# Pyrokine/LineSegmentDetector-SLAM

Measured on NVIDIA B200. Metric: lsd_source_mpixel_per_s, higher is better.
Workload: dtype f64

## Files before the change

include/lsdb200.h:

```cpp
#ifndef LSDB200_H
#define LSDB200_H
#include <stdint.h>

#ifdef __cplusplus
extern "C" {
#endif

#define LSDB_OK 0
#define LSDB_ERR_CUDA 1
#define LSDB_ERR_ARG 2
#define LSDB_ERR_CAPACITY 3
#define LSDB_ERR_TIMEOUT 4
#define LSDB_ERR_NO_DEVICE 5

#define LSDB_MAX_ANGLE 524288.0

typedef struct lsdb_ctx lsdb_ctx;
typedef struct lsdb_batch lsdb_batch;
typedef struct lsdb_fa_map lsdb_fa_map;

typedef struct {
    double sca;
    double sig;
    double angThre;
    double denThre;
    int pseBin;
    int _pad;
} lsdb_lsd_params;

typedef struct {
    double k, b, dx, dy, x1, y1, x2, y2, len;
    int orient;
    int _pad;
} lsdb_line;

typedef struct {
    double x1, y1, x2, y2, wid, cX, cY, deg, dx, dy, p, prec, logNFA;
} lsdb_rect;

enum { LSDB_STAGE_STENCIL = 0, LSDB_STAGE_ORDER = 1, LSDB_STAGE_GROW = 2, LSDB_NSTAGES = 3 };

typedef struct {
    long long cells, live_seeds, grows, grown_px, small, regrows, rrr_passes, nfa_calls, nfa_px,
        rejects, accepts, spec_evals, respec_evals, chunks;
    long long cyc_grow, cyc_rect, cyc_nfa, cyc_wait, cyc_retire, cyc_spec, cyc_respec;
    long long cyc_map, ns_map, spare_;
    long long rs_none, rs_conflict, rs_commit, rs_lost_commit, rs_pad[4];
} lsdb_stats;

int lsdb_create(lsdb_ctx** out, int device, void* stream);
int lsdb_set_team_warps(lsdb_ctx* ctx, int warps);
void lsdb_destroy(lsdb_ctx* ctx);
const char* lsdb_last_error(const lsdb_ctx* ctx);
const char* lsdb_version(void);

int lsdb_batch_create(lsdb_ctx* ctx, int n_maps, const int* cols, const int* rows,
                      const lsdb_lsd_params* params, int max_lines_per_map, lsdb_batch** out);
void lsdb_batch_destroy(lsdb_batch* b);
int lsdb_batch_upload(lsdb_batch* b, const uint8_t* const* maps);
int lsdb_batch_run(lsdb_batch* b);
int lsdb_batch_sync(lsdb_batch* b);
int lsdb_batch_download(lsdb_batch* b, int* counts, lsdb_line* lines, lsdb_rect* rects);
int lsdb_batch_line_image(lsdb_batch* b, int i, uint8_t* line_im);
int lsdb_batch_line_images(lsdb_batch* b, uint8_t* const* line_ims);
int lsdb_batch_planes(lsdb_batch* b, int i, double* mag, double* deg, uint8_t* used, int32_t* labels,
                      int32_t* seeds, int max_seeds, int* n_seeds, double* max_grad);
int lsdb_batch_stage_ms(lsdb_batch* b, float* ms );
int lsdb_batch_stats(lsdb_batch* b, lsdb_stats* total);
int lsdb_batch_map_stats(lsdb_batch* b, int i, lsdb_stats* out);
int lsdb_batch_launches(const lsdb_batch* b);
// ... 100 lines not shown
```

linesegmentdetector-slam_b200/__init__.py:

```python
import ctypes as C
import os
import numpy as np

HERE = os.path.dirname(os.path.abspath(__file__))
SO_PATH = os.path.join(HERE, "liblsdb200.so")
LSD_DEFAULTS = dict(sca=0.3, sig=0.6, angThre=22.5, denThre=0.7, pseBin=1024)
ERR_NAMES = {1: "CUDA", 2: "ARG", 3: "CAPACITY", 4: "TIMEOUT", 5: "NO_DEVICE"}
STAGES = ("stencil", "order", "grow")
STAT_FIELDS = ["cells", "live_seeds", "grows", "grown_px", "small", "regrows", "rrr_passes", "nfa_calls", "nfa_px",
               "rejects", "accepts", "spec_evals", "respec_evals", "chunks", "cyc_grow", "cyc_rect", "cyc_nfa", "cyc_wait",
               "cyc_retire", "cyc_spec", "cyc_respec", "cyc_map", "ns_map", "spare_", "rs_none", "rs_conflict", "rs_commit", "rs_lost_commit", "rs_pad0", "rs_pad1", "rs_pad2", "rs_pad3"]

LINE_DTYPE = np.dtype([("k", "f8"), ("b", "f8"), ("dx", "f8"), ("dy", "f8"), ("x1", "f8"), ("y1", "f8"), ("x2", "f8"),
                       ("y2", "f8"), ("len", "f8"), ("orient", "i4"), ("_pad", "i4")])
RECT_FIELDS = ["x1", "y1", "x2", "y2", "wid", "cX", "cY", "deg", "dx", "dy", "p", "prec", "logNFA"]
EST_DTYPE = np.dtype([("n_hyp", "i4"), ("n_kept", "i4"), ("best_x", "f8"), ("best_y", "f8"), ("best_ang", "f8"), ("best_score", "f8"),
                      ("mean_x", "f8"), ("mean_y", "f8"), ("mean_ang", "f8"), ("mean_score", "f8")])
SCAN_INFO_DTYPE = np.dtype([("n_lines", "i4"), ("n_pts", "i4"), ("im_cols", "i4"), ("im_rows", "i4"), ("lidar_x", "f8"), ("lidar_y", "f8")])
RDP_DEFAULTS = dict(least_point=3, thre_line=0.08, least_dist_m=0.5)
HYP_DTYPE = np.dtype([("frame", "i4"), ("i_scan", "i4"), ("i_map", "i4"), ("i_pair", "i4"), ("x", "f8"), ("y", "f8"),
                      ("ang", "f8"), ("score", "f8")])
LEGACY_EST_DTYPE = np.dtype([("n_cols", "i4"), ("best_col", "i4"), ("best_score", "f8"), ("estimate_pose", "f8", (3,)),
                             ("estimate_pose_realworld", "f8", (3,))])


class LsdbError(RuntimeError):
    pass


class _Params(C.Structure):
    _fields_ = [("sca", C.c_double), ("sig", C.c_double), ("angThre", C.c_double), ("denThre", C.c_double),
                ("pseBin", C.c_int), ("_pad", C.c_int)]


# ... 510 lines not shown
```

linesegmentdetector-slam_b200/csrc/api.cu:

```cuda
#include "../../include/lsdb200.h"
#include "lsdb_common.cuh"

#include <limits.h>
#include <stdio.h>
#include <stdlib.h>
#include <string.h>
#include <algorithm>
#include <math.h>
#include <string>
#include <vector>

struct lsdb_ctx {
    int device;
    cudaStream_t stream;
    bool ownStream;
    std::string err;
    double* lgammaTab;
    int lgammaN;
    int maxGrowCtas;
    int teamWarps;
    lsdb_batch* cached;
    cudaEvent_t faEv[2];
    float faMs;
    void* faDev; size_t faDevCap;
    void* faHost; size_t faHostCap;
    void* faAux; void* faAuxHost; size_t faAuxCap;
    void* faIn; size_t faInCap;
    void* faInHost; size_t faInHostCap;
    void* faKeep; size_t faKeepCap;
    void* fsOut; void* fsOutHost; size_t fsOutCap, fsOutHostCap;
    void* fsLinesDev; void* fsPtsDev;
    void* fsIm; size_t fsImCap;
    void* fsTmp; size_t fsTmpCap;
    float fsMs;
};

struct lsdb_batch {
    lsdb_ctx* ctx;
    int n;
    lsdb_lsd_params params;
    int maxSeg, listCap, arenaCap, nTiles, nCtas, nWarps, runAhead, bmCapWords, steal, stencilMode;
    size_t totalN, totalSrc, totalBan;
    std::vector<LsdbImg> imgs;
    LsdbLsdConst kc;
    uint8_t* src; double* mag; double* deg; double* cosm; double* sinm; unsigned int* state; unsigned short* bins; unsigned int* cells;
    int* labels; LsdbRect* rects; LsdbImgDyn* dyn; LsdbImg* imgsD; int* tileImg; unsigned int* lists;
    int* imgCounter; LsdbLsdConst* kcD; double* gaussDbg; unsigned char* recBuf; unsigned int* banBits;
    uint8_t* lineImD;
    double* mcCache;
    unsigned int* nzBits; int2* bandOf; int2* bandsOfImg; unsigned int* orderTabs; int nBands;
    LsdbImgDyn* dynH; LsdbRect* rectsH;
    cudaEvent_t ev[4];
    bool ran, downloaded, mcReady;
    int launches;
};

static int fail(lsdb_ctx* c, int code, const char* fmt, const char* a = "", long long v = 0) {
    char buf[512];
    snprintf(buf, sizeof buf, fmt, a, v);
    if (c) c->err = buf;
    return code;
}
#define CK(ctx, call)                                                                         \
    do {                                                                                      \
// ... 180 lines not shown
        int sms = 148;
        cudaDeviceGetAttribute(&sms, cudaDevAttrMultiProcessorCount, ctx->device);
        int bmMax = lsdb_grow_max_bitmap_words(ctx->device);
        int bmLimit = 48 * 1024 / 4;
        if (getenv("LSDB_SMEM_BAN_KB")) bmLimit = atoi(getenv("LSDB_SMEM_BAN_KB")) * 1024 / 4;
        if (bmMax > bmLimit) bmMax = bmLimit;
        b->bmCapWords = maxBanWords <= bmMax ? maxBanWords : 0;
        if (getenv("LSDB_NO_SMEM_BAN")) b->bmCapWords = 0;
        int nw = 1184 / n;
        if (nw > LSDB_GROW_WARPS) nw = LSDB_GROW_WARPS;
        const int sizeCap = maxN < 30000 ? 4 : 8;
        if (nw > sizeCap) nw = sizeCap;
        if (nw < 1) nw = 1;
        if (ctx->teamWarps > 0) nw = ctx->teamWarps;
        if (getenv("LSDB_GROW_WARPS")) { int v = atoi(getenv("LSDB_GROW_WARPS")); if (v >= 1 && v <= LSDB_GROW_WARPS) nw = v; }
        b->nWarps = nw;
        if (nw == 1 && !getenv("LSDB_SMEM_BAN_KB")) b->bmCapWords = 0;
        b->runAhead = 0;
        if (getenv("LSDB_RUNAHEAD")) b->runAhead = atoi(getenv("LSDB_RUNAHEAD"));
        b->stencilMode = lsdb_stencil_mode();
        b->steal = 0;
        if (getenv("LSDB_STEAL")) b->steal = atoi(getenv("LSDB_STEAL")) & 0xff;
        if (getenv("LSDB_SUPER_SHIFT")) b->steal |= ((atoi(getenv("LSDB_SUPER_SHIFT")) & 3) + 1) << 8;
        const int maxCtas = lsdb_grow_max_ctas(ctx->device, nw, b->bmCapWords);
        b->nCtas = n < maxCtas ? n : maxCtas;
        if (getenv("LSDB_GROW_CTAS")) { int v = atoi(getenv("LSDB_GROW_CTAS")); if (v >= 1 && v < b->nCtas) b->nCtas = v; }
        (void)sms;
    }

    cudaError_t e = cudaSuccess;
#define AL(ptr, bytes) if (e == cudaSuccess) e = cudaMalloc((void**)&(ptr), (bytes))
    AL(b->src, b->totalSrc + 64); AL(b->mag, b->totalN * 8); AL(b->deg, b->totalN * 8); AL(b->cosm, b->totalN * 16 + 16);    AL(b->state, b->totalN * 4);
    AL(b->bins, b->totalN * 2); AL(b->cells, b->totalN * 4); AL(b->labels, b->totalN * 4);
    AL(b->rects, (size_t)n * b->maxSeg * sizeof(LsdbRect)); AL(b->dyn, (size_t)n * sizeof(LsdbImgDyn));
    AL(b->imgsD, (size_t)n * sizeof(LsdbImg)); AL(b->tileImg, (size_t)b->nTiles * sizeof(int));
    b->arenaCap = 8 * b->listCap < (1 << 14) ? (1 << 14) : (8 * b->listCap > (1 << 16) ? (1 << 16) : 8 * b->listCap);
    AL(b->lists, (size_t)b->nCtas * lsdb_grow_words_per_cta(b->listCap, b->arenaCap, b->nWarps) * 4);
    AL(b->recBuf, (size_t)b->nCtas * lsdb_grow_rec_bytes_per_cta());
    AL(b->imgCounter, 64); AL(b->kcD, sizeof(LsdbLsdConst)); AL(b->banBits, (b->totalBan + 4) * 4); AL(b->nzBits, (b->totalBan + 4) * 4);
    std::vector<int2> bandOfH, bandsOfImgH(n);
    {
        int sms = 148;
        cudaDeviceGetAttribute(&sms, cudaDevAttrMultiProcessorCount, ctx->device);
        int K = (12 * sms + n - 1) / n;
        for (int i = 0; i < n; i++) {
            int k = K;
// ... 33 lines not shown
    for (int i = 0; i < b->n; i++) {
        const LsdbImg& im = b->imgs[i];
        CK(ctx, cudaMemcpy2DAsync(b->src + im.srcOff, im.srcPitch, maps[i], im.cols, im.cols, im.rows, cudaMemcpyHostToDevice, ctx->stream));
    }
    return LSDB_OK;
}

extern "C" int lsdb_batch_run(lsdb_batch* b) {
    if (!b) return LSDB_ERR_ARG;
    lsdb_ctx* ctx = b->ctx;
    cudaStream_t s = ctx->stream;
    CK(ctx, cudaSetDevice(ctx->device));
    CK(ctx, cudaMemsetAsync(b->dyn, 0, (size_t)b->n * sizeof(LsdbImgDyn), s));
    CK(ctx, cudaMemsetAsync(b->labels, 0, b->totalN * 4, s));
    CK(ctx, cudaMemsetAsync(b->imgCounter, 0, 64, s));
    CK(ctx, cudaEventRecord(b->ev[0], s));
    const int nStencil = lsdb_launch_stencil(s, b->nTiles, b->imgsD, b->tileImg, b->dyn, b->kcD, b->src, b->mag, b->deg, b->cosm, b->sinm, b->state, b->banBits, b->nzBits, b->gaussDbg, 0,
                        b->cells, b->totalN * 4, b->imgCounter + 8, b->stencilMode);
    CK(ctx, cudaEventRecord(b->ev[1], s));
    lsdb_launch_order(s, b->n, b->nBands, b->imgsD, b->dyn, b->kcD, b->mag, b->nzBits, b->bandOf, b->bandsOfImg, b->orderTabs, b->bins, b->cells);
    CK(ctx, cudaEventRecord(b->ev[2], s));
    lsdb_launch_grow(s, b->n, b->nCtas, b->nWarps, b->imgsD, b->dyn, b->kcD, b->mag, b->deg, b->cosm, b->sinm, b->state, b->cells, b->labels, b->rects,
                     b->maxSeg, b->lists, b->listCap, b->arenaCap, b->runAhead, b->recBuf, ctx->lgammaTab, ctx->lgammaN, b->imgCounter, b->banBits,
                     b->bmCapWords, b->steal);
    CK(ctx, cudaEventRecord(b->ev[3], s));
    CK(ctx, cudaGetLastError());
    b->ran = true; b->downloaded = false; b->launches = 4 + nStencil;
    return LSDB_OK;
}

extern "C" int lsdb_batch_launches(const lsdb_batch* b) { return b ? b->launches : 0; }

extern "C" int lsdb_batch_run_stencil_rows(lsdb_batch* b, int tileRow0, int tileRow1) {
    if (!b) return LSDB_ERR_ARG;
    lsdb_ctx* ctx = b->ctx;
    if (b->n != 1) return fail(ctx, LSDB_ERR_ARG, "lsdb_batch_run_stencil_rows: single-map batches only%s");
    const LsdbImg& im = b->imgs[0];
    if (tileRow0 < 0 || tileRow1 > im.tilesY || tileRow0 > tileRow1) return fail(ctx, LSDB_ERR_ARG, "lsdb_batch_run_stencil_rows: bad tile-row range%s");
    cudaStream_t s = ctx->stream;
    CK(ctx, cudaSetDevice(ctx->device));
    CK(ctx, cudaMemsetAsync(b->dyn, 0, sizeof(LsdbImgDyn), s));
    CK(ctx, cudaMemsetAsync(b->labels, 0, b->totalN * 4, s));
    CK(ctx, cudaMemsetAsync(b->imgCounter, 0, 64, s));
    CK(ctx, cudaEventRecord(b->ev[0], s));
    const int nStencil = lsdb_launch_stencil(s, (tileRow1 - tileRow0) * im.tilesX, b->imgsD, b->tileImg, b->dyn, b->kcD, b->src, b->mag, b->deg, b->cosm, b->sinm, b->state,
                        b->banBits, b->nzBits, b->gaussDbg, tileRow0 * im.tilesX, b->cells, b->totalN * 4, b->imgCounter + 8, b->stencilMode);
    CK(ctx, cudaEventRecord(b->ev[1], s));
// ... 17 lines not shown
    const LsdbImg& im = b->imgs[0];
    ptrs[0] = b->mag + im.nOff; rowBytes[0] = 8ll * im.W;
    ptrs[1] = b->deg + im.nOff; rowBytes[1] = 8ll * im.W;
    ptrs[2] = b->cosm + 2 * im.nOff; rowBytes[2] = 16ll * im.W;
    ptrs[3] = b->state + im.nOff; rowBytes[3] = 4ll * im.W;
    ptrs[4] = b->banBits + im.banOff; rowBytes[4] = 4ll * im.pw;
    ptrs[5] = b->nzBits + im.banOff; rowBytes[5] = 4ll * im.pw;
    *nPlanes = 6;
    if (tileRows) *tileRows = im.tilesY;
    if (rowsPerTile) *rowsPerTile = LSDB_TILE;
    return LSDB_OK;
}

extern "C" int lsdb_batch_run_regions(lsdb_batch* b) {
    if (!b) return LSDB_ERR_ARG;
    lsdb_ctx* ctx = b->ctx;
    cudaStream_t s = ctx->stream;
    CK(ctx, cudaSetDevice(ctx->device));
    CK(ctx, cudaEventRecord(b->ev[1], s));
    lsdb_launch_order(s, b->n, b->nBands, b->imgsD, b->dyn, b->kcD, b->mag, b->nzBits, b->bandOf, b->bandsOfImg, b->orderTabs, b->bins, b->cells);
    CK(ctx, cudaEventRecord(b->ev[2], s));
    lsdb_launch_grow(s, b->n, b->nCtas, b->nWarps, b->imgsD, b->dyn, b->kcD, b->mag, b->deg, b->cosm, b->sinm, b->state, b->cells, b->labels, b->rects,
                     b->maxSeg, b->lists, b->listCap, b->arenaCap, b->runAhead, b->recBuf, ctx->lgammaTab, ctx->lgammaN, b->imgCounter, b->banBits,
                     b->bmCapWords, b->steal);
    CK(ctx, cudaEventRecord(b->ev[3], s));
    CK(ctx, cudaGetLastError());
    b->ran = true; b->downloaded = false; b->launches += 4;
    return LSDB_OK;
}

static int fetch_dyn(lsdb_batch* b) {
    lsdb_ctx* ctx = b->ctx;
    CK(ctx, cudaSetDevice(ctx->device));
    CK(ctx, cudaMemcpyAsync(b->dynH, b->dyn, (size_t)b->n * sizeof(LsdbImgDyn), cudaMemcpyDeviceToHost, ctx->stream));
    CK(ctx, cudaStreamSynchronize(ctx->stream));
    for (int i = 0; i < b->n; i++) {
        if (b->dynH[i].err == LSDB_ERR_TIMEOUT) return fail(ctx, LSDB_ERR_TIMEOUT, "map %s%lld: ordered-commit watchdog fired", "", i);
        if (b->dynH[i].err) return fail(ctx, LSDB_ERR_CAPACITY, "map %s%lld: region list or segment capacity exceeded", "", i);
    }
    return LSDB_OK;
}

extern "C" int lsdb_batch_sync(lsdb_batch* b) {
    if (!b) return LSDB_ERR_ARG;
    if (!b->ran) return fail(b->ctx, LSDB_ERR_ARG, "lsdb_batch_sync before lsdb_batch_run%s");
    return fetch_dyn(b);
}
// ... 805 lines not shown
```

linesegmentdetector-slam_b200/csrc/grow.cu:

```cuda
#include "lsdb_common.cuh"
#include "../../include/lsdb200.h"
#include <stdlib.h>

#define NW_MAX LSDB_GROW_WARPS
#define ARENA_HDR 32
#define GRID 32
#define FULL 0xffffffffu

enum { OC_NONE = 0, OC_NOCHANGE = 1, OC_REJECT = 2, OC_ACCEPT = 3, OC_DEFER = 4 };
enum { ST_CELLS = 0, ST_LIVE, ST_GROWS, ST_GROWNPX, ST_SMALL, ST_REGROWS, ST_RRR, ST_NFACALLS, ST_NFAPX, ST_REJECTS,
       ST_ACCEPTS, ST_SPEC, ST_RESPEC, ST_CHUNKS, ST_N,
       TM_GROW = ST_N, TM_RECT, TM_NFA, TM_WAIT, TM_RETIRE, TM_SPEC, TM_RESPEC, TM_MAPCYC, TM_MAPNS, TM_SPARE, RS_NONE, RS_CONFLICT, RS_COMMIT, RS_LOST, RS_P0, RS_P1, RS_P2, RS_P3, TM_N };

#define RING 512
#define NSLOTS (RING / LSDB_SUPER)
#define LQ_CAP 256
#define SG_CAP 32
struct GrowShared {
    volatile int frontier;
    int nextChunk;
    int runAhead;
    int supShift;
    int retireLock;
    volatile int nSeg;
    volatile int abortFlag;
    int img;
    int nChunks;
    int nCells;
    volatile int chunkFlag[RING];
    volatile unsigned char chunkHeavy[RING];
    volatile int chunkSeen[RING];
    unsigned int slotHead[NSLOTS];
    volatile int slotPending[NSLOTS];
    volatile unsigned int lq[LQ_CAP][2];
    volatile unsigned int lqReady[LQ_CAP];
// ... 36 lines not shown
    const double* cosm;
    const double* sinm;
    unsigned int* list;
    unsigned int* scratch;
    unsigned int* arenas;
    unsigned int* q;
    int listCap, arenaCap;
    const LsdbLsdConst* kc;
    const double* lgammaTab;
    int lgammaN;
    GrowShared* sh;
    unsigned int* rej[2];
    int rejCap;
    unsigned int* pnd;
    int npnd;
    int steal;
    int specChunk;
    double* stage;
    volatile unsigned int* bm;
    bool bmInSmem;
    int pw;
    double logNT, regThre;
    int cellShift;
};

__device__ __forceinline__ void bbox_add(const WarpCtx& c, BBox& b, int x, int y) {
    b.x0 = min(b.x0, x); b.y0 = min(b.y0, y); b.x1 = max(b.x1, x); b.y1 = max(b.y1, y);
}

__device__ __noinline__ double d_sin(double x) { return lsdm_sin(x); }
__device__ __noinline__ double d_cos(double x) { return lsdm_cos(x); }
__device__ __noinline__ double d_atan2(double y, double x) { return lsdm_atan2(y, x); }
__device__ __noinline__ double d_log(double x) { return lsdm_log(x); }
__device__ __noinline__ double d_log10(double x) { return lsdm_log10(x); }
__device__ __noinline__ double d_exp(double x) { return lsdm_exp(x); }
__device__ __noinline__ double d_pow(double x, double y) { return lsdm_pow(x, y); }

__device__ __forceinline__ unsigned int pack_xy(int x, int y) { return ((unsigned int)y << 16) | (unsigned int)x; }
__device__ __forceinline__ int px_of(unsigned int v) { return (int)(v & 0xffffu); }
__device__ __forceinline__ int py_of(unsigned int v) { return (int)(v >> 16); }


__device__ void clear_bits(const WarpCtx& c, const unsigned int* lst, int num) {
    for (int k = c.lane; k < num; k += 32) {
        unsigned int v = lst[k];
        atomicAnd(&c.state[(size_t)py_of(v) * c.W + px_of(v)], ~c.mybit);
// ... 366 lines not shown
                        if (pass) {
                            lst[num] = pk;
                            rej[num] = 0;
                            num++;
                            mine |= sg_bit(n, m);
                            cosS += cd;
                            sinS += sd;
                            if (num >= T) running = false;
                            else {
                                n2 = cosS * cosS + sinS * sinS;
                                c2n2 = c2 * n2; m2 = 4e-13 * n2; nrmOK = n2 > 1e-18;
                            }
                        } else {
                            nr |= 1u << nb;
                        }
                    }
                }
            }
        }
    }
    return num;
}

__device__ __noinline__ Rect rect_from_region(const WarpCtx& c, const unsigned int* lst, int num, double regDeg, double aliPro,
                                 double degThre) {
    const int W = c.W;
    const double pi = c.kc->pi;
    TIC;
    double* stg = c.stage;
    double acc = 0.0;
    for (int base = 0; base < num; base += 32) {
        const int k = base + c.lane;
        const unsigned int v = k < num ? lst[k] : 0u;
        const double wv = k < num ? c.mag[(size_t)py_of(v) * W + px_of(v)] : 0.0;
        stg[c.lane * 4 + 0] = wv * px_of(v);
        stg[c.lane * 4 + 1] = wv * py_of(v);
        stg[c.lane * 4 + 2] = wv;
        __syncwarp();
        const int cnt = min(32, num - base);
        if (c.lane < 3)
            for (int j = 0; j < cnt; j++) acc += stg[j * 4 + c.lane];
        __syncwarp();
    }
    double cenX = __shfl_sync(FULL, acc, 0), cenY = __shfl_sync(FULL, acc, 1), weiSum = __shfl_sync(FULL, acc, 2);
    cenX = cenX / weiSum;
    cenY = cenY / weiSum;
// ... 554 lines not shown
    GrowShared& sh = *c.sh;
    unsigned int p = 0, ci = 0;
    int got = 0;
    if (c.lane == 0) {
        while (true) {
            const unsigned int h = *(volatile unsigned int*)&sh.lqHead;
            if (h == *(volatile unsigned int*)&sh.lqTail) break;
            const int e = h & (LQ_CAP - 1);
            if (sh.lqReady[e] != h + 1) break;
            p = sh.lq[e][0]; ci = sh.lq[e][1];
            if (atomicCAS(&sh.lqHead, h, h + 1) == h) { got = 1; break; }
        }
    }
    got = __shfl_sync(FULL, got, 0);
    if (!got) return false;
    p = __shfl_sync(FULL, p, 0); ci = __shfl_sync(FULL, ci, 0);
    eval_large(c, (int)p, (int)ci, R);
    __threadfence();
    if (c.lane == 0) atomicSub((int*)&sh.slotPending[slot_of_chunk(sh, (int)ci >> 5)], 1);
    __syncwarp();
    return true;
}

__device__ void speculate_super(WarpCtx& c, int chunk0, int nSub, const unsigned int* cl, int nCells, const ChunkRecs& R, int T) {
    GrowShared& sh = *c.sh;
    const int lane = c.lane;
    const unsigned int lt = (1u << lane) - 1u;
    long long tSpec = clock64();
    const int slot = slot_of_chunk(*c.sh, chunk0);
    unsigned int* q = c.q;
    int qn = 0;
    for (int s = 0; s < nSub; s++) {
        const int ci = (chunk0 + s) * LSDB_CHUNK + lane;
        const int p = ci < nCells ? (int)cl[ci] : -1;
        const bool live = p >= 0 && !seed_taken(lsdb_ld_state(&c.state[p]), chunk0 + s);
        const unsigned int bal = __ballot_sync(FULL, live);
        if (live) {
            const int k = qn + __popc(bal & lt);
            q[2 * k] = (unsigned int)p;
            q[2 * k + 1] = (unsigned int)((s << 5) | lane);
        }
        qn += __popc(bal);
        R.oc[(size_t)((chunk0 + s) & (RING - 1)) * 32 + lane] = OC_NONE;
    }
    if (lane < nSub) { sh.chunkHeavy[(chunk0 + lane) & (RING - 1)] = 0; sh.chunkSeen[(chunk0 + lane) & (RING - 1)] = -1; }
    __syncwarp();
    for (int base = 0; base < qn && !aborted(c); base += 32) {
        const int k = base + lane;
        bool act = k < qn;
        const unsigned int rel = act ? q[2 * k + 1] : 0u;
        const int myChunk = chunk0 + (int)(rel >> 5);
        const int myp = act ? (int)q[2 * k] : 0;
        if (act && seed_taken(lsdb_ld_state(&c.state[myp]), myChunk)) act = false;
        unsigned int lst[SG_CAP];
        unsigned int pnd[SG_PND];
        int num = 0, npnd = 0;
        bool large = act;
        const int L0 = sh.nSeg;
        __threadfence_block();
        if (T <= SG_CAP && c.kc->degThre <= c.kc->pi / 2.0) {
            num = small_grow(c, act, myp, T, lst, myChunk, pnd, npnd);
            large = act && num >= T;
        }
        __syncwarp();
        const bool small = act && !large && npnd >= 0;
        const int need = small ? num + npnd : 0;
        int incl = need;
#pragma unroll
        for (int o = 1; o < 32; o <<= 1) {
            const int t = __shfl_up_sync(FULL, incl, o);
            if (lane >= o) incl += t;
        }
        const int tot = __shfl_sync(FULL, incl, 31);
        const int off = tot > 0 ? slot_alloc(c, slot, tot) : -1;
        if (small && off >= 0) {
            const size_t ri = (size_t)(myChunk & (RING - 1)) * 32 + (rel & 31u);
            BBox sb; sb.x0 = sb.y0 = 0x7fffffff; sb.x1 = sb.y1 = -1;
            const int mine = off + (incl - need);
            unsigned int* dst = c.arenas + (size_t)slot * c.arenaCap + mine;
            for (int j = 0; j < num; j++) { dst[j] = lst[j]; bbox_add(c, sb, px_of(lst[j]), py_of(lst[j])); }
            for (int j = 0; j < npnd; j++) dst[num + j] = pnd[j];
            R.L0[ri] = L0; R.b0[ri] = pack_xy(sb.x0, sb.y0); R.b1[ri] = pack_xy(sb.x1, sb.y1); 
            R.off[ri] = 0; R.chk[ri] = num; R.chkOff[ri] = (unsigned int)mine;
            R.pnd[ri] = npnd; R.pndOff[ri] = (unsigned int)(mine + num);
// ... 221 lines not shown
            atomicAdd(&sh.stats[ST_CHUNKS], 1ull);
            __threadfence_block();
            sh.frontier = f + 1;
        }
        __syncwarp();
    }
    if (c.lane == 0) {
        atomicAdd(&sh.stats[TM_RETIRE], (unsigned long long)(clock64() - t0));
        __threadfence_block();
        atomicExch(&sh.retireLock, 0);
    }
    __syncwarp();
}

template <int MAXT>
__global__ void __launch_bounds__(MAXT, 1) lsdb_grow_kernel(int nImgs, const LsdbImg* __restrict__ imgs, LsdbImgDyn* __restrict__ dyn,
                                                                   const LsdbLsdConst* __restrict__ kc, const double* __restrict__ mag,
                                                                   const double* __restrict__ deg, const double* __restrict__ cosm,
                                                                   const double* __restrict__ sinm, unsigned int* __restrict__ state,
                                                                   const unsigned int* __restrict__ cells, int* __restrict__ labels,
                                                                   LsdbRect* __restrict__ rects, int maxSeg, unsigned int* __restrict__ lists,
                                                                   int listCap, int arenaCap, int runAhead, unsigned char* __restrict__ recBuf,
                                                                   const double* __restrict__ lgammaTab, int lgammaN, int* __restrict__ imgCounter,
                                                                   unsigned int* banBits, int bmCapWords, int steal) {
    __shared__ GrowShared sh;
    extern __shared__ unsigned int bmShared[];
    const int tid = threadIdx.x, lane = tid & 31, w = tid >> 5, nw = blockDim.x >> 5;
    WarpCtx c;
    c.lane = lane; c.w = w; c.mybit = 1u << (LSDB_ST_WARP_SHIFT + w);
    c.kc = kc; c.lgammaTab = lgammaTab; c.lgammaN = lgammaN; c.sh = &sh;
    c.listCap = listCap; c.arenaCap = arenaCap;
    c.rejCap = LSDB_REJ_CAP;
    c.arenas = lists + (size_t)blockIdx.x * grow_words_per_cta(listCap, arenaCap, nw);
    c.list = c.arenas + (size_t)NSLOTS * arenaCap + (size_t)w * grow_words_per_warp(listCap);
    c.scratch = c.list + listCap;
    c.rej[0] = c.scratch + 2 * (size_t)listCap + 64;
    c.rej[1] = c.rej[0] + LSDB_REJ_CAP;
    c.pnd = c.rej[1] + LSDB_REJ_CAP; c.npnd = 0; c.specChunk = -1;
    c.q = c.pnd + LSDB_PND_CAP;
    c.steal = steal & 0xff;
    c.stage = reinterpret_cast<double*>(bmShared + ((bmCapWords + 1) & ~1)) + (size_t)w * 128;
    ChunkRecs R;
    {
        unsigned char* base = recBuf + (size_t)blockIdx.x * (RING * 32 * REC_BYTES_PER_CELL);
        R.mask = reinterpret_cast<unsigned long long*>(base);
        R.oc = reinterpret_cast<int*>(base + RING * 32 * 8);
        R.L0 = R.oc + RING * 32; R.b0 = reinterpret_cast<unsigned int*>(R.L0 + RING * 32); R.b1 = R.b0 + RING * 32;
// ... 30 lines not shown
        long long mapC0 = 0; unsigned long long mapT0 = 0;
        if (tid == 0) { mapC0 = clock64(); asm volatile("mov.u64 %0, %%globaltimer;" : "=l"(mapT0)); }
        const LsdbImg im = imgs[img];
        c.W = im.W; c.H = im.H; c.logNT = im.logNT; c.regThre = im.regThre;
        {
            int k = 0;
            while (((max(im.W, im.H) - 1) >> k) > GRID - 1) k++;
            c.cellShift = k;
        }
        c.state = state + im.nOff; c.deg = deg + im.nOff; c.mag = mag + im.nOff; c.cosm = cosm + 2 * im.nOff; c.sinm = sinm + 2 * im.nOff;
        c.pw = im.pw;
        {
            const int words = im.H * im.pw;
            if (words <= bmCapWords) {
                const unsigned int* srcB = banBits + im.banOff;
                for (int i = tid; i < words; i += blockDim.x) bmShared[i] = srcB[i];
                c.bm = bmShared; c.bmInSmem = true;
            } else {
                c.bm = banBits + im.banOff; c.bmInSmem = false;
            }
        }
        const int T = (int)ceil(im.regThre);
        __syncthreads();
        int* lab = labels + im.nOff;
        const unsigned int* cl = cells + im.nOff;
        LsdbRect* rc = rects + im.segOff;
        const int nCells = sh.nCells, nChunks = sh.nChunks;
        unsigned int idle = 0;

        while (!aborted(c)) {
            try_retire(c, cl, nCells, nChunks, R, lab, rc, maxSeg);
            if (__shfl_sync(FULL, (int)sh.frontier, 0) >= nChunks) break;
            int chunk = -1;
            if (lane == 0) {
                if (sh.nextChunk < nChunks && sh.nextChunk - sh.frontier < sh.runAhead) {
                    chunk = atomicAdd(&sh.nextChunk, 1 << sh.supShift);
                    if (chunk >= nChunks) chunk = -1;
                    else { sh.slotHead[slot_of_chunk(sh, chunk)] = 0; sh.slotPending[slot_of_chunk(sh, chunk)] = 0; }
                }
            }
            chunk = __shfl_sync(FULL, chunk, 0);
            if (chunk < 0) {
                if (help_large(c, R)) { idle = 0; continue; }
                if (revalidate_ahead(c, cl, nCells, nChunks, R)) { idle = 0; continue; }
                long long tw = clock64();
                __nanosleep(200);
// ... 17 lines not shown
        }
        __syncthreads();
        if (tid < TM_N) dyn[img].stat[tid] = (long long)sh.stats[tid];
    }
}

__global__ void lsdb_used_plane_kernel(const unsigned int* __restrict__ state, uint8_t* __restrict__ used, int n) {
    int i = blockIdx.x * blockDim.x + threadIdx.x;
    if (i < n) {
        unsigned int s = state[i];
        used[i] = (s & LSDB_ST_BAN) ? 1 : ((s & LSDB_ST_REJ) ? 2 : 0);
    }
}

static bool lsdb_grow_wide_regs(int nCtas, int warpsPerCta) {
    if (getenv("LSDB_GROW_WIDE")) return atoi(getenv("LSDB_GROW_WIDE")) != 0 && warpsPerCta <= 8;
    return warpsPerCta <= 8 && nCtas <= 148;
}

void lsdb_launch_grow(cudaStream_t s, int nImgs, int nCtas, int warpsPerCta, const LsdbImg* imgs, LsdbImgDyn* dyn,
                      const LsdbLsdConst* kc, const double* mag, const double* deg, const double* cosm, const double* sinm,
                      unsigned int* state, const unsigned int* cells, int* labels, LsdbRect* rects, int maxSeg,
                      unsigned int* lists, int listCap, int arenaCap, int runAhead, unsigned char* recBuf, const double* lgammaTab, int lgammaN,
                      int* imgCounter, unsigned int* banBits, int bmCapWords, int steal) {
    if (runAhead <= 0 || runAhead > RING - (NW_MAX + 1) * LSDB_SUPER) runAhead = RING - (NW_MAX + 1) * LSDB_SUPER;
    if (runAhead < 1) runAhead = 1;
    const bool wide = lsdb_grow_wide_regs(nCtas, warpsPerCta);
    if (wide) cudaFuncSetAttribute(lsdb_grow_kernel<256>, cudaFuncAttributeMaxDynamicSharedMemorySize, (int)grow_dyn_smem(bmCapWords, NW_MAX));
    else cudaFuncSetAttribute(lsdb_grow_kernel<NW_MAX * 32>, cudaFuncAttributeMaxDynamicSharedMemorySize, (int)grow_dyn_smem(bmCapWords, NW_MAX));
    if (nImgs <= 0) return;
    if (wide)
        lsdb_grow_kernel<256><<<nCtas, warpsPerCta * 32, grow_dyn_smem(bmCapWords, warpsPerCta), s>>>(
            nImgs, imgs, dyn, kc, mag, deg, cosm, sinm, state, cells, labels, rects, maxSeg, lists, listCap, arenaCap, runAhead, recBuf,
            lgammaTab, lgammaN, imgCounter, banBits, bmCapWords, steal);
    else
        lsdb_grow_kernel<NW_MAX * 32><<<nCtas, warpsPerCta * 32, grow_dyn_smem(bmCapWords, warpsPerCta), s>>>(
            nImgs, imgs, dyn, kc, mag, deg, cosm, sinm, state, cells, labels, rects, maxSeg, lists, listCap, arenaCap, runAhead, recBuf,
            lgammaTab, lgammaN, imgCounter, banBits, bmCapWords, steal);
}

size_t lsdb_grow_words_per_cta(int listCap, int arenaCap, int warpsPerCta) { return grow_words_per_cta(listCap, arenaCap, warpsPerCta); }
size_t lsdb_grow_rec_bytes_per_cta(void) { return (size_t)RING * 32 * REC_BYTES_PER_CELL; }


void lsdb_launch_lgamma_table(cudaStream_t s, double* tab, int n) {
    lsdb_lgamma_table_kernel<<<(n + 127) / 128, 128, 0, s>>>(tab, n);
}

void lsdb_launch_used_plane(cudaStream_t s, const unsigned int* state, uint8_t* used, int n) {
    lsdb_used_plane_kernel<<<(n + 255) / 256, 256, 0, s>>>(state, used, n);
}

int lsdb_grow_max_ctas(int device, int warpsPerCta, int bmCapWords) {
    int sms = 0, per = 0;
    cudaDeviceGetAttribute(&sms, cudaDevAttrMultiProcessorCount, device);
    cudaFuncSetAttribute(lsdb_grow_kernel<NW_MAX * 32>, cudaFuncAttributeMaxDynamicSharedMemorySize, (int)grow_dyn_smem(bmCapWords, NW_MAX));
    cudaOccupancyMaxActiveBlocksPerMultiprocessor(&per, lsdb_grow_kernel<NW_MAX * 32>, warpsPerCta * 32, grow_dyn_smem(bmCapWords, warpsPerCta));
    if (per < 1) per = 1;
    return sms * per;
}

// ... 9 lines not shown
```

linesegmentdetector-slam_b200/csrc/lsdb_common.cuh:

```cuda
#pragma once
#include <cuda_runtime.h>
#include <stdint.h>
#include "lsd_math.h"

struct LsdbImg {
    int cols, rows;
    int W, H;
    int n;
    int srcPitch;
    int tile0;
    int tilesX, tilesY;
    int pw;
    unsigned long long banOff;
    unsigned long long srcOff;
    unsigned long long nOff;
    unsigned long long segOff;
    double logNT;
    double regThre;
};

struct LsdbImgDyn {
    unsigned long long maxGradBits;
    int nCells;
    int nSeg;
// ... 40 lines not shown
    return __double2int_rz(v);
}
#endif

int lsdb_stencil_mode(void);
int lsdb_launch_stencil(cudaStream_t s, int nTiles, const LsdbImg* imgs, const int* tileImg, LsdbImgDyn* dyn,
                         const LsdbLsdConst* kc, const uint8_t* src, double* mag, double* deg, double* cosm, double* sinm,
                         unsigned int* state, unsigned int* banBits, unsigned int* nzBits, double* gaussOut, int tileBase,
                         void* deferBuf, size_t deferBytes, int* deferCount, int mode);
int lsdb_launch_stencil_v2(cudaStream_t s, int nTiles, const LsdbImg* imgs, const int* tileImg, LsdbImgDyn* dyn,
                            const LsdbLsdConst* kc, const uint8_t* src, double* mag, double* deg, double* cosm, double* sinm,
                            unsigned int* state, unsigned int* banBits, unsigned int* nzBits, double* gaussOut, int tileBase,
                            void* deferBuf, size_t deferBytes, int* deferCount, int groups);
void lsdb_launch_order(cudaStream_t s, int nImgs, int nBands, const LsdbImg* imgs, LsdbImgDyn* dyn, const LsdbLsdConst* kc,
                       const double* mag, const unsigned int* nzBits, const int2* bandOf, const int2* bandsOfImg, unsigned int* tabs,
                       unsigned short* bins, unsigned int* cells);
size_t lsdb_order_tab_words_per_band(void);
void lsdb_launch_line_images(cudaStream_t s, int nImgs, int maxSeg, const LsdbImg* imgs, const LsdbImgDyn* dyn, const LsdbRect* rects,
                             uint8_t* plane);
void lsdb_launch_grow(cudaStream_t s, int nImgs, int nCtas, int warpsPerCta, const LsdbImg* imgs, LsdbImgDyn* dyn,
                      const LsdbLsdConst* kc, const double* mag, const double* deg, const double* cosm, const double* sinm,
                      unsigned int* state, const unsigned int* cells, int* labels, LsdbRect* rects, int maxSeg,
                      unsigned int* lists, int listCap, int arenaCap, int runAhead, unsigned char* recBuf, const double* lgammaTab, int lgammaN,
                      int* imgCounter, unsigned int* banBits, int bmCapWords, int steal);
size_t lsdb_grow_rec_bytes_per_cta(void);
size_t lsdb_grow_words_per_cta(int listCap, int arenaCap, int warpsPerCta);
void lsdb_launch_lgamma_table(cudaStream_t s, double* tab, int n);
void lsdb_launch_used_plane(cudaStream_t s, const unsigned int* state, uint8_t* used, int n);
int lsdb_grow_max_ctas(int device, int warpsPerCta, int bmCapWords);
int lsdb_grow_max_bitmap_words(int device);

struct LsdbFaTask { int frame, iScan, iMap, pad; };
struct LsdbFaHyp { int frame, iScan, iMap, iPair; double x, y, ang, score; };
struct LsdbFaLine { double k, b, dx, dy, x1, y1, x2, y2, len; int orient, pad; };
void lsdb_launch_fa(cudaStream_t s, int nTasks, const LsdbFaTask* tasks, const LsdbFaLine* scanLines, const int* scanLineOff,
                    const double* pts, const int* ptOff, const double* lidarPose, const double* lastPose,
                    const LsdbFaLine* mapLines, const double* mapCache, int cols, int rows, double pi, LsdbFaHyp* out, void* poseBuf);
size_t lsdb_fa_pose_bytes(int nTasks);
struct LsdbFaEst { int nHyp, nKept; double bx, by, bang, bscore, mx, my, mang, mscore; };
void lsdb_launch_fa_reduce(cudaStream_t s, int nFrames, const LsdbFaHyp* hyp, const int* hypOff, LsdbFaEst* est);
struct LsdbFaLegacyEst { int nCols, bestCol; double bestScore, pose[3], real[3]; };
void lsdb_launch_fa_legacy(cudaStream_t s, int nHyp, const LsdbFaTask* tasks, const LsdbFaLine* scanLines, const int* scanLineOff,
                           const LsdbFaLine* mapLines, const int* lidarPos, const double* mapCache, int cols, int rows, double resol,
                           const double* ranges, const double* angles, const int* rayOff, double* out);
void lsdb_launch_fa_legacy_reduce(cudaStream_t s, int nFrames, const int* colOff, const double* rec, double resol, double oriX, double oriY,
                                  LsdbFaLegacyEst* est);
size_t lsdb_fa_pairs_scratch_ints(int nL);
// ... 20 lines not shown
```

Before: 22720.

## Pre-scout small regions per image before grow to skip tiny-region growth

Adds a prescout pass at the start of each image in the grow kernel. It runs a capped small_grow, or a single-pixel neighbour test, over all unbanned pixels and stores a compact 16-bit code for regions of at most four pixels in a per-pixel buffer (reusing b->bins). During speculation, seeds with a valid code are resolved directly as no-change outcomes, after checking that their pixels are not banned or pending, instead of being queued for growth. This trades an upfront pass over every unbanned pixel for skipping many serial small grows, and it risks stale codes, which is why an optional check mode exists.

```diff
diff --git a/include/lsdb200.h b/include/lsdb200.h
--- a/include/lsdb200.h
+++ b/include/lsdb200.h
@@ -44,8 +44,9 @@
     long long cells, live_seeds, grows, grown_px, small, regrows, rrr_passes, nfa_calls, nfa_px,
         rejects, accepts, spec_evals, respec_evals, chunks;
     long long cyc_grow, cyc_rect, cyc_nfa, cyc_wait, cyc_retire, cyc_spec, cyc_respec;
-    long long cyc_map, ns_map, spare_;
-    long long rs_none, rs_conflict, rs_commit, rs_lost_commit, rs_pad[4];
+    long long cyc_map, ns_map, cyc_small_grow;
+    long long rs_none, rs_conflict, rs_commit, rs_lost_commit;
+    long long ps_decided, ps_fallback, ps_mismatch, cyc_prescout;
 } lsdb_stats;
 
 int lsdb_create(lsdb_ctx** out, int device, void* stream);
diff --git a/linesegmentdetector-slam_b200/__init__.py b/linesegmentdetector-slam_b200/__init__.py
--- a/linesegmentdetector-slam_b200/__init__.py
+++ b/linesegmentdetector-slam_b200/__init__.py
@@ -9,7 +9,8 @@
 STAGES = ("stencil", "order", "grow")
 STAT_FIELDS = ["cells", "live_seeds", "grows", "grown_px", "small", "regrows", "rrr_passes", "nfa_calls", "nfa_px",
                "rejects", "accepts", "spec_evals", "respec_evals", "chunks", "cyc_grow", "cyc_rect", "cyc_nfa", "cyc_wait",
-               "cyc_retire", "cyc_spec", "cyc_respec", "cyc_map", "ns_map", "spare_", "rs_none", "rs_conflict", "rs_commit", "rs_lost_commit", "rs_pad0", "rs_pad1", "rs_pad2", "rs_pad3"]
+               "cyc_retire", "cyc_spec", "cyc_respec", "cyc_map", "ns_map", "cyc_small_grow", "rs_none", "rs_conflict", "rs_commit", "rs_lost_commit", "ps_decided", "ps_fallback",
+               "ps_mismatch", "cyc_prescout"]
 
 LINE_DTYPE = np.dtype([("k", "f8"), ("b", "f8"), ("dx", "f8"), ("dy", "f8"), ("x1", "f8"), ("y1", "f8"), ("x2", "f8"),
                        ("y2", "f8"), ("len", "f8"), ("orient", "i4"), ("_pad", "i4")])
diff --git a/linesegmentdetector-slam_b200/csrc/api.cu b/linesegmentdetector-slam_b200/csrc/api.cu
--- a/linesegmentdetector-slam_b200/csrc/api.cu
+++ b/linesegmentdetector-slam_b200/csrc/api.cu
@@ -40,6 +40,7 @@
     int n;
     lsdb_lsd_params params;
     int maxSeg, listCap, arenaCap, nTiles, nCtas, nWarps, runAhead, bmCapWords, steal, stencilMode;
+    int prescout;
     size_t totalN, totalSrc, totalBan;
     std::vector<LsdbImg> imgs;
     LsdbLsdConst kc;
@@ -266,6 +267,10 @@
         b->steal = 0;
         if (getenv("LSDB_STEAL")) b->steal = atoi(getenv("LSDB_STEAL")) & 0xff;
         if (getenv("LSDB_SUPER_SHIFT")) b->steal |= ((atoi(getenv("LSDB_SUPER_SHIFT")) & 3) + 1) << 8;
+        b->prescout = 4;
+        if (getenv("LSDB_PRESCOUT") && atoi(getenv("LSDB_PRESCOUT")) == 0) b->prescout = 0;
+        else if (getenv("LSDB_PRESCOUT_K")) { int v = atoi(getenv("LSDB_PRESCOUT_K")); b->prescout = v < 0 ? 0 : (v > 4 ? 4 : v); }
+        if (b->prescout && getenv("LSDB_PRESCOUT_CHECK") && atoi(getenv("LSDB_PRESCOUT_CHECK")) != 0) b->prescout |= 1 << 8;
         const int maxCtas = lsdb_grow_max_ctas(ctx->device, nw, b->bmCapWords);
         b->nCtas = n < maxCtas ? n : maxCtas;
         if (getenv("LSDB_GROW_CTAS")) { int v = atoi(getenv("LSDB_GROW_CTAS")); if (v >= 1 && v < b->nCtas) b->nCtas = v; }
@@ -345,7 +350,7 @@
     CK(ctx, cudaEventRecord(b->ev[2], s));
     lsdb_launch_grow(s, b->n, b->nCtas, b->nWarps, b->imgsD, b->dyn, b->kcD, b->mag, b->deg, b->cosm, b->sinm, b->state, b->cells, b->labels, b->rects,
                      b->maxSeg, b->lists, b->listCap, b->arenaCap, b->runAhead, b->recBuf, ctx->lgammaTab, ctx->lgammaN, b->imgCounter, b->banBits,
-                     b->bmCapWords, b->steal);
+                     b->bmCapWords, b->steal, b->bins, b->prescout);
     CK(ctx, cudaEventRecord(b->ev[3], s));
     CK(ctx, cudaGetLastError());
     b->ran = true; b->downloaded = false; b->launches = 4 + nStencil;
@@ -409,7 +414,7 @@
     CK(ctx, cudaEventRecord(b->ev[2], s));
     lsdb_launch_grow(s, b->n, b->nCtas, b->nWarps, b->imgsD, b->dyn, b->kcD, b->mag, b->deg, b->cosm, b->sinm, b->state, b->cells, b->labels, b->rects,
                      b->maxSeg, b->lists, b->listCap, b->arenaCap, b->runAhead, b->recBuf, ctx->lgammaTab, ctx->lgammaN, b->imgCounter, b->banBits,
-                     b->bmCapWords, b->steal);
+                     b->bmCapWords, b->steal, b->bins, b->prescout);
     CK(ctx, cudaEventRecord(b->ev[3], s));
     CK(ctx, cudaGetLastError());
     b->ran = true; b->downloaded = false; b->launches += 4;
diff --git a/linesegmentdetector-slam_b200/csrc/grow.cu b/linesegmentdetector-slam_b200/csrc/grow.cu
--- a/linesegmentdetector-slam_b200/csrc/grow.cu
+++ b/linesegmentdetector-slam_b200/csrc/grow.cu
@@ -10,7 +10,8 @@
 enum { OC_NONE = 0, OC_NOCHANGE = 1, OC_REJECT = 2, OC_ACCEPT = 3, OC_DEFER = 4 };
 enum { ST_CELLS = 0, ST_LIVE, ST_GROWS, ST_GROWNPX, ST_SMALL, ST_REGROWS, ST_RRR, ST_NFACALLS, ST_NFAPX, ST_REJECTS,
        ST_ACCEPTS, ST_SPEC, ST_RESPEC, ST_CHUNKS, ST_N,
-       TM_GROW = ST_N, TM_RECT, TM_NFA, TM_WAIT, TM_RETIRE, TM_SPEC, TM_RESPEC, TM_MAPCYC, TM_MAPNS, TM_SPARE, RS_NONE, RS_CONFLICT, RS_COMMIT, RS_LOST, RS_P0, RS_P1, RS_P2, RS_P3, TM_N };
+       TM_GROW = ST_N, TM_RECT, TM_NFA, TM_WAIT, TM_RETIRE, TM_SPEC, TM_RESPEC, TM_MAPCYC, TM_MAPNS, TM_SMALL, RS_NONE, RS_CONFLICT, RS_COMMIT, RS_LOST,
+       PS_DECIDED, PS_FALLBACK, PS_MISMATCH, TM_PRESCOUT, TM_N };
 
 #define RING 512
 #define NSLOTS (RING / LSDB_SUPER)
@@ -93,6 +94,8 @@
     int pw;
     double logNT, regThre;
     int cellShift;
+    unsigned short* codes;
+    bool psCheck;
 };
 
 __device__ __forceinline__ void bbox_add(const WarpCtx& c, BBox& b, int x, int y) {
@@ -505,6 +508,139 @@
     return num;
 }
 
+#define PS_UNDECIDED 0u
+#define PS_SINGLE 1u
+#define PS_SMALL 2u
+#define PS_MAXK 4
+
+__device__ __forceinline__ unsigned int ps_encode(const unsigned int* lst, int num) {
+    if (num == 1) return PS_SINGLE;
+    const int sx = px_of(lst[0]), sy = py_of(lst[0]);
+    const int i9 = (py_of(lst[1]) - sy + 1) * 3 + (px_of(lst[1]) - sx + 1);
+    unsigned int code = PS_SMALL | (unsigned int)(i9 - (i9 > 4)) << 2;
+    code |= (num > 2 ? (unsigned int)((py_of(lst[2]) - sy + 2) * 5 + (px_of(lst[2]) - sx + 2)) : 31u) << 5;
+    code |= (num > 3 ? (unsigned int)((py_of(lst[3]) - sy + 3) * 7 + (px_of(lst[3]) - sx + 3)) : 63u) << 10;
+    return code;
+}
+__device__ __forceinline__ int ps_decode(unsigned int code, int sx, int sy, unsigned int* px) {
+    px[0] = pack_xy(sx, sy);
+    if ((code & 3u) != PS_SMALL) return 1;
+    int i9 = (code >> 2) & 7u;
+    i9 += i9 >= 4;
+    px[1] = pack_xy(sx + i9 % 3 - 1, sy + i9 / 3 - 1);
+    const unsigned int i25 = (code >> 5) & 31u, i49 = code >> 10;
+    if (i25 >= 25u) return 2;
+    px[2] = pack_xy(sx + (int)(i25 % 5u) - 2, sy + (int)(i25 / 5u) - 2);
+    if (i49 >= 49u) return 3;
+    px[3] = pack_xy(sx + (int)(i49 % 7u) - 3, sy + (int)(i49 / 7u) - 3);
+    return 4;
+}
+
+__device__ void prescout_single_batch(const WarpCtx& c, const unsigned int* q, int n);
+
+__device__ void prescout_batch(const WarpCtx& c, const unsigned int* q, int n, int cap) {
+    if (cap == 2) { prescout_single_batch(c, q, n); return; }
+    const bool act = c.lane < n;
+    const int p = act ? (int)q[c.lane] : 0;
+    unsigned int lst[SG_CAP];
+    unsigned int pnd[SG_PND];
+    int npnd = 0;
+    const int num = small_grow(c, act, p, cap, lst, -1, pnd, npnd);
+    if (act) c.codes[p] = (unsigned short)(num < cap ? ps_encode(lst, num) : PS_UNDECIDED);
+    __syncwarp();
+}
+
+__device__ void prescout_single_batch(const WarpCtx& c, const unsigned int* q, int n) {
+    if (c.lane < n) {
+        const int W = c.W;
+        const int p0 = (int)q[c.lane];
+        const int sx = p0 % W, sy = p0 / W;
+        const unsigned int cm = (~ban9(c, sx, sy)) & 0x1efu;
+        const double pi = c.kc->pi, pi32 = pi * 3 / 2.0, pi2 = 2.0 * pi;
+        const double degThre = c.kc->degThre, cTau = c.kc->cosDegThre;
+        const double c2 = cTau * cTau;
+        const double cosS = c.cosm[2 * (size_t)p0], sinS = c.sinm[2 * (size_t)p0];
+        const double n2 = cosS * cosS + sinS * sinS, c2n2 = c2 * n2, m2 = 4e-13 * n2;
+        const bool nrmOK = n2 > 1e-18;
+        double cd[9], sd[9];
+#pragma unroll
+        for (int nb = 0; nb < 9; nb++) {
+            cd[nb] = 0.0; sd[nb] = 0.0;
+            if ((cm >> nb) & 1u) {
+                const size_t p = (size_t)(sy + nb / 3 - 1) * W + (sx + nb % 3 - 1);
+                cd[nb] = c.cosm[2 * p]; sd[nb] = c.sinm[2 * p];
+            }
+        }
+        bool single = true;
+#pragma unroll
+        for (int nb = 0; nb < 9; nb++) {
+            if ((cm >> nb) & 1u) {
+                const double dot = cosS * cd[nb] + sinS * sd[nb];
+                const double d2 = dot * dot - c2n2;
+                bool pass = dot > 0 && d2 > 0;
+                if ((dot > 0 && !(fabs(d2) > m2)) || !nrmOK) {
+                    const size_t p = (size_t)(sy + nb / 3 - 1) * W + (sx + nb % 3 - 1);
+                    double degDif = fabs(c.deg[p0] - c.deg[p]);
+                    if (degDif > pi32) degDif = fabs(degDif - pi2);
+                    pass = degDif < degThre;
+                }
+                if (pass) single = false;
+            }
+        }
+        c.codes[p0] = (unsigned short)(single ? PS_SINGLE : PS_UNDECIDED);
+    }
+    __syncwarp();
+}
+
+__device__ void prescout_map(const WarpCtx& c, int nw, int cap) {
+    const int lane = c.lane;
+    const int nWords = c.H * c.pw;
+    unsigned int* q = c.q;
+    static_assert(LSDB_Q_WORDS >= 16 * 32, "a block of ban words must fit the queue");
+    int pend = 0;
+    for (int blk = c.w; blk * 16 < nWords; blk += nw) {
+        const int wi = blk * 16 + lane;
+        unsigned int m = 0;
+        int base = 0;
+        if (lane < 16 && wi < nWords) {
+            const int y = wi / c.pw, x0 = (wi - y * c.pw) * 32;
+            if (x0 < c.W) {
+                m = ~c.bm[wi];
+                if (c.W - x0 < 32) m &= (1u << (c.W - x0)) - 1u;
+            }
+            base = y * c.W + x0;
+        }
+        const int cnt = __popc(m);
+        int incl = cnt;
+#pragma unroll
+        for (int o = 1; o < 16; o <<= 1) {
+            const int t = __shfl_up_sync(FULL, incl, o);
+            if (lane >= o) incl += t;
+        }
+        const int total = __shfl_sync(FULL, incl, 15);
+        if (total == 0) continue;
+        if (pend + total > LSDB_Q_WORDS) { prescout_batch(c, q, pend, cap); pend = 0; }
+        int o = pend + incl - cnt;
+        while (m) {
+            const int b = __ffs(m) - 1;
+            m &= m - 1;
+            q[o++] = (unsigned int)(base + b);
+        }
+        __syncwarp();
+        pend += total;
+        int done = 0;
+        for (; pend - done >= 32; done += 32) prescout_batch(c, q + done, 32, cap);
+        if (done) {
+            const unsigned int v = lane < pend - done ? q[done + lane] : 0u;
+            __syncwarp();
+            if (lane < pend - done) q[lane] = v;
+            __syncwarp();
+            pend -= done;
+        }
+    }
+    if (pend) prescout_batch(c, q, pend, cap);
+}
+
 __device__ __noinline__ Rect rect_from_region(const WarpCtx& c, const unsigned int* lst, int num, double regDeg, double aliPro,
                                  double degThre) {
     const int W = c.W;
@@ -1105,6 +1241,20 @@
     return true;
 }
 
+__device__ void ps_check(const WarpCtx& c, int p, const unsigned int* lst, int num, const unsigned int* pnd, int npnd) {
+    unsigned int px[PS_MAXK];
+    const int n = ps_decode(c.codes[p], p % c.W, p / c.W, px);
+    bool same = num == n;
+    for (int j = 0; j < n && j < num; j++) same = same && lst[j] == px[j];
+    if (same) return;
+    bool moved = npnd < 0;
+    for (int j = 0; j < n; j++) {
+        moved = moved || (lsdb_ld_state(&c.state[(size_t)py_of(px[j]) * c.W + px_of(px[j])]) & LSDB_ST_BAN);
+        for (int i = 0; i < npnd; i++) moved = moved || pnd[i] == px[j];
+    }
+    if (!moved) atomicAdd(&c.sh->stats[PS_MISMATCH], 1ull);
+}
+
 __device__ void speculate_super(WarpCtx& c, int chunk0, int nSub, const unsigned int* cl, int nCells, const ChunkRecs& R, int T) {
     GrowShared& sh = *c.sh;
     const int lane = c.lane;
@@ -1113,25 +1263,78 @@
     const int slot = slot_of_chunk(*c.sh, chunk0);
     unsigned int* q = c.q;
     int qn = 0;
+    const int L0 = sh.nSeg;
+    __threadfence_block();
     for (int s = 0; s < nSub; s++) {
-        const int ci = (chunk0 + s) * LSDB_CHUNK + lane;
+        const int chunkS = chunk0 + s;
+        const int ci = chunkS * LSDB_CHUNK + lane;
         const int p = ci < nCells ? (int)cl[ci] : -1;
-        const bool live = p >= 0 && !seed_taken(lsdb_ld_state(&c.state[p]), chunk0 + s);
-        const unsigned int bal = __ballot_sync(FULL, live);
-        if (live) {
+        const bool live = p >= 0 && !seed_taken(lsdb_ld_state(&c.state[p]), chunkS);
+        const size_t ri = (size_t)(chunkS & (RING - 1)) * 32 + lane;
+        int oc = OC_NONE;
+        bool dec = false, reGrow = false;
+        if (c.codes) {
+            const unsigned int code = live ? c.codes[p] : PS_UNDECIDED;
+            unsigned int px[PS_MAXK];
+            int n = 0;
+            if (code & 3u) {
+                n = ps_decode(code, p % c.W, p / c.W, px);
+                dec = true;
+                for (int j = 1; j < n; j++) {
+                    const unsigned int st = lsdb_ld_state(&c.state[(size_t)py_of(px[j]) * c.W + px_of(px[j])]);
+                    if ((st & LSDB_ST_BAN) || pend_applies(st, LSDB_ST_PACC, chunkS)) dec = false;
+                }
+            }
+            const int need = dec && n > 1 ? n : 0;
+            int incl = need;
+#pragma unroll
+            for (int o = 1; o < 32; o <<= 1) {
+                const int t = __shfl_up_sync(FULL, incl, o);
+                if (lane >= o) incl += t;
+            }
+            const int tot = __shfl_sync(FULL, incl, 31);
+            const int off = tot > 0 ? slot_alloc(c, slot, tot) : -1;
+            if (need && off < 0) dec = false;
+            if (dec) {
+                const int mine = need ? off + (incl - need) : 0;
+                unsigned int* dst = c.arenas + (size_t)slot * c.arenaCap + mine;
+                BBox sb; sb.x0 = sb.y0 = 0x7fffffff; sb.x1 = sb.y1 = -1;
+                for (int j = 0; j < n; j++) { if (need) dst[j] = px[j]; bbox_add(c, sb, px_of(px[j]), py_of(px[j])); }
+                R.L0[ri] = L0; R.b0[ri] = pack_xy(sb.x0, sb.y0); R.b1[ri] = pack_xy(sb.x1, sb.y1);
+                R.off[ri] = 0; R.chk[ri] = need; R.chkOff[ri] = (unsigned int)mine;
+                R.pnd[ri] = 0; R.pndOff[ri] = (unsigned int)mine;
+                oc = OC_NOCHANGE;
+            }
+            reGrow = dec && c.psCheck;
+            const unsigned int nDec = __popc(__ballot_sync(FULL, dec));
+            const unsigned int nFall = __popc(__ballot_sync(FULL, (code & 3u) && !dec));
+            int pxs = dec ? n : 0;
+#pragma unroll
+            for (int o = 16; o > 0; o >>= 1) pxs += __shfl_xor_sync(FULL, pxs, o);
+            if (lane == 0 && (nDec | nFall)) {
+                atomicAdd(&sh.stats[ST_SPEC], (unsigned long long)nDec); atomicAdd(&sh.stats[ST_GROWS], (unsigned long long)nDec);
+                atomicAdd(&sh.stats[ST_SMALL], (unsigned long long)nDec); atomicAdd(&sh.stats[ST_GROWNPX], (unsigned long long)pxs);
+                atomicAdd(&sh.stats[PS_DECIDED], (unsigned long long)nDec); atomicAdd(&sh.stats[PS_FALLBACK], (unsigned long long)nFall);
+            }
+        }
+        const bool enq = (live && !dec) || reGrow;
+        const unsigned int bal = __ballot_sync(FULL, enq);
+        if (enq) {
             const int k = qn + __popc(bal & lt);
             q[2 * k] = (unsigned int)p;
-            q[2 * k + 1] = (unsigned int)((s << 5) | lane);
+            q[2 * k + 1] = (unsigned int)((s << 5) | lane) | (reGrow ? 0x80000000u : 0u);
         }
         qn += __popc(bal);
-        R.oc[(size_t)((chunk0 + s) & (RING - 1)) * 32 + lane] = OC_NONE;
+        R.oc[ri] = oc;
     }
     if (lane < nSub) { sh.chunkHeavy[(chunk0 + lane) & (RING - 1)] = 0; sh.chunkSeen[(chunk0 + lane) & (RING - 1)] = -1; }
     __syncwarp();
     for (int base = 0; base < qn && !aborted(c); base += 32) {
         const int k = base + lane;
         bool act = k < qn;
-        const unsigned int rel = act ? q[2 * k + 1] : 0u;
+        unsigned int rel = act ? q[2 * k + 1] : 0u;
+        const bool reGrow = rel >> 31;
+        rel &= 0x7fffffffu;
         const int myChunk = chunk0 + (int)(rel >> 5);
         const int myp = act ? (int)q[2 * k] : 0;
         if (act && seed_taken(lsdb_ld_state(&c.state[myp]), myChunk)) act = false;
@@ -1142,7 +1345,13 @@
         const int L0 = sh.nSeg;
         __threadfence_block();
         if (T <= SG_CAP && c.kc->degThre <= c.kc->pi / 2.0) {
+            const long long tSg = clock64();
             num = small_grow(c, act, myp, T, lst, myChunk, pnd, npnd);
+            if (lane == 0) atomicAdd(&sh.stats[TM_SMALL], (unsigned long long)(clock64() - tSg));
+            if (reGrow) {
+                if (act) ps_check(c, myp, lst, num, pnd, npnd);
+                act = false;
+            }
             large = act && num >= T;
         }
         __syncwarp();
@@ -1410,7 +1619,8 @@
                                                                    LsdbRect* __restrict__ rects, int maxSeg, unsigned int* __restrict__ lists,
                                                                    int listCap, int arenaCap, int runAhead, unsigned char* __restrict__ recBuf,
                                                                    const double* __restrict__ lgammaTab, int lgammaN, int* __restrict__ imgCounter,
-                                                                   unsigned int* banBits, int bmCapWords, int steal) {
+                                                                   unsigned int* banBits, int bmCapWords, int steal,
+                                                                   unsigned short* __restrict__ codes, int prescout) {
     __shared__ GrowShared sh;
     extern __shared__ unsigned int bmShared[];
     const int tid = threadIdx.x, lane = tid & 31, w = tid >> 5, nw = blockDim.x >> 5;
@@ -1487,6 +1697,18 @@
         }
         const int T = (int)ceil(im.regThre);
         __syncthreads();
+        {
+            const int K = prescout & 0xff;
+            const int cap = min(K + 1, T);
+            c.codes = codes && K > 0 && cap >= 2 && T <= SG_CAP && kc->degThre <= kc->pi / 2.0 ? codes + im.nOff : nullptr;
+            c.psCheck = (prescout >> 8) & 1;
+            if (c.codes) {
+                const long long t0 = clock64();
+                prescout_map(c, nw, cap);
+                if (lane == 0) atomicAdd(&sh.stats[TM_PRESCOUT], (unsigned long long)(clock64() - t0));
+                __syncthreads();
+            }
+        }
         int* lab = labels + im.nOff;
         const unsigned int* cl = cells + im.nOff;
         LsdbRect* rc = rects + im.segOff;
@@ -1550,7 +1772,7 @@
                       const LsdbLsdConst* kc, const double* mag, const double* deg, const double* cosm, const double* sinm,
                       unsigned int* state, const unsigned int* cells, int* labels, LsdbRect* rects, int maxSeg,
                       unsigned int* lists, int listCap, int arenaCap, int runAhead, unsigned char* recBuf, const double* lgammaTab, int lgammaN,
-                      int* imgCounter, unsigned int* banBits, int bmCapWords, int steal) {
+                      int* imgCounter, unsigned int* banBits, int bmCapWords, int steal, unsigned short* codes, int prescout) {
     if (runAhead <= 0 || runAhead > RING - (NW_MAX + 1) * LSDB_SUPER) runAhead = RING - (NW_MAX + 1) * LSDB_SUPER;
     if (runAhead < 1) runAhead = 1;
     const bool wide = lsdb_grow_wide_regs(nCtas, warpsPerCta);
@@ -1560,11 +1782,11 @@
     if (wide)
         lsdb_grow_kernel<256><<<nCtas, warpsPerCta * 32, grow_dyn_smem(bmCapWords, warpsPerCta), s>>>(
             nImgs, imgs, dyn, kc, mag, deg, cosm, sinm, state, cells, labels, rects, maxSeg, lists, listCap, arenaCap, runAhead, recBuf,
-            lgammaTab, lgammaN, imgCounter, banBits, bmCapWords, steal);
+            lgammaTab, lgammaN, imgCounter, banBits, bmCapWords, steal, codes, prescout);
     else
         lsdb_grow_kernel<NW_MAX * 32><<<nCtas, warpsPerCta * 32, grow_dyn_smem(bmCapWords, warpsPerCta), s>>>(
             nImgs, imgs, dyn, kc, mag, deg, cosm, sinm, state, cells, labels, rects, maxSeg, lists, listCap, arenaCap, runAhead, recBuf,
-            lgammaTab, lgammaN, imgCounter, banBits, bmCapWords, steal);
+            lgammaTab, lgammaN, imgCounter, banBits, bmCapWords, steal, codes, prescout);
 }
 
 size_t lsdb_grow_words_per_cta(int listCap, int arenaCap, int warpsPerCta) { return grow_words_per_cta(listCap, arenaCap, warpsPerCta); }
diff --git a/linesegmentdetector-slam_b200/csrc/lsdb_common.cuh b/linesegmentdetector-slam_b200/csrc/lsdb_common.cuh
--- a/linesegmentdetector-slam_b200/csrc/lsdb_common.cuh
+++ b/linesegmentdetector-slam_b200/csrc/lsdb_common.cuh
@@ -86,7 +86,8 @@
                       const LsdbLsdConst* kc, const double* mag, const double* deg, const double* cosm, const double* sinm,
                       unsigned int* state, const unsigned int* cells, int* labels, LsdbRect* rects, int maxSeg,
                       unsigned int* lists, int listCap, int arenaCap, int runAhead, unsigned char* recBuf, const double* lgammaTab, int lgammaN,
-                      int* imgCounter, unsigned int* banBits, int bmCapWords, int steal);
+                      int* imgCounter, unsigned int* banBits, int bmCapWords, int steal,
+                      unsigned short* codes, int prescout);
 size_t lsdb_grow_rec_bytes_per_cta(void);
 size_t lsdb_grow_words_per_cta(int listCap, int arenaCap, int warpsPerCta);
 void lsdb_launch_lgamma_table(cudaStream_t s, double* tab, int n);
```

Result: slower. 21060 (median of 6 runs) (-7.3%).
